# pyg-team/pytorch_geometric

Measured on AMD Instinct MI355X. Metric: edges/sec (fwd+bwd) 3-layer SAGE, ogbn-products shape, higher is better.
Workload: dtype f32

## Files before the change

pytorch_geometric_amd/_native.py:

```python
import collections
import ctypes
import os
import threading
from typing import Optional, Tuple

import torch
from torch import Tensor

from . import _compiled, _lib
from ._lib import REDUCE_IDS, PygAmdError, SpmmArgs, check

HUB_THRESHOLD = 1024
HUB_CHUNK = int(os.environ.get('PYGAMD_HUB_CHUNK', '256'))


def _require_device(*tensors):
    for t in tensors:
        if t is not None and not t.is_cuda:
            raise PygAmdError(
                'pytorch_geometric_amd kernels need HIP device tensors (got a '
                f'{t.device} tensor); there is no CPU fallback on this path')


def _idx_dtype(t: Tensor) -> int:
# ... 1375 lines not shown


SAGE_FUSED_VARIANT = int(os.environ.get('PYGAMD_FUSED_VARIANT', '0'))
SAGE_FUSED_PROBE = 0
AGG_GIVEN = _lib.AGG_GIVEN


def sage_layer_forward(rowptr: Tensor, col: Tensor, x_gather: Tensor, x_root: Tensor, w: Tensor,
                       bias: Optional[Tensor], reduce: str, relu: bool, agg: Tensor, out: Tensor,
                       hub=None, save_agg=True, hub_threshold: int = None,
                       hub_chunk: int = None, relu_bits: Optional[Tensor] = None,
                       mask_bits: Optional[Tensor] = None, row_scale: Optional[Tensor] = None,
                       out_scaled: Optional[Tensor] = None, variant: Optional[int] = None,
                       gather_width: Optional[int] = None,
                       compressed_out: Optional[Tensor] = None,
                       rowend: Optional[Tensor] = None) -> Tensor:
    _require_device(rowptr, col, x_gather, x_root, w, bias, agg, out, relu_bits, mask_bits,
                    row_scale, out_scaled, compressed_out)
    variant = SAGE_FUSED_VARIANT if variant is None else variant
    given = not isinstance(save_agg, bool) and int(save_agg) == AGG_GIVEN
    save_agg = AGG_GIVEN if given else int(bool(save_agg))
    if given:
        if gather_width is not None:
            raise ValueError("'save_agg=AGG_GIVEN' reads dense aggregated rows: not with a "
                             "compressed 'x_gather'")
        hub = None
    lab = bool(variant or SAGE_FUSED_PROBE)
    C = None if lab else _compiled.ops()
    if (C is not None and gather_width is None and compressed_out is None and rowend is None
            and _plain(x_gather, x_root, w, agg, out, out_scaled)):
        n_rows, F, Fo = rowptr.numel() - 1, x_gather.size(1), w.size(0)
        ok = (x_root.shape == (n_rows, F) and w.size(1) == 2 * F and agg.shape == (n_rows, F)
              and out.shape == (n_rows, Fo)
              and (out_scaled is None or (row_scale is not None and row_scale.numel() == n_rows
                                          and row_scale.dtype == torch.float32
                                          and out_scaled.shape == (n_rows, Fo)
                                          and (Fo <= 1 or out_scaled.stride(1) == 1))))
        if ok:
            _check_bits(relu_bits, n_rows, Fo)
            _check_bits(mask_bits, n_rows, Fo)
            h_rows, h_cptr, n_hub, n_chunks = _hub4(hub)
            with _timed({'n_rows': n_rows, 'n_src': x_gather.size(0),
                         'nnz': 0 if given else col.numel(), 'F': F,
                         'reduce': reduce, 'idx_bytes': rowptr.element_size(), 'weighted': False,
                         'src_scale': False, 'accumulate': False, 'n_hub': n_hub,
                         'fused_gemm': {'Fo': Fo, 'K': 2 * F, 'save_agg': bool(save_agg),
                                        'backward': mask_bits is not None,
                                        'scaled_copy': out_scaled is not None}}, x_gather):
                if given:
                    C.sage_layer_given(rowptr, x_root, w, bias, REDUCE_IDS[reduce], relu, agg,
                                       out, relu_bits, mask_bits, row_scale, out_scaled)
                else:
                    C.sage_layer_fused(
                        rowptr, col, x_gather, x_root, w, bias, REDUCE_IDS[reduce], relu, agg,
                        out, h_rows, h_cptr, n_hub, n_chunks,
                        HUB_THRESHOLD if hub_threshold is None else hub_threshold,
                        HUB_CHUNK if hub_chunk is None else hub_chunk, save_agg, relu_bits,
                        mask_bits, row_scale, out_scaled)
            return out
    lib = _lib.load_lab() if lab else _lib.load()
    xr, w2 = _f32_rows(x_root, 'x_root'), _f32_rows(w, 'weight')
    if gather_width is None:
        xg = _f32_rows(x_gather, 'x')
        F = xg.size(1)
    else:
        _check_compressed(x_gather, gather_width, 'x_gather')
        xg, F = x_gather, gather_width
    n_rows, Fo = rowptr.numel() - 1, w2.size(0)
    if rowend is not None:
        _require_device(rowend)
        n_rows = xr.size(0)
        if rowend.dtype != rowptr.dtype or not rowend.is_contiguous() \
                or rowend.numel() < n_rows or rowptr.numel() < n_rows:
            raise ValueError("'rowend' needs the dtype of 'rowptr' and one entry per row")
    if xr.shape != (n_rows, F) or w2.size(1) != 2 * F or agg.shape != (n_rows, F) \
            or out.shape != (n_rows, Fo):
        raise ValueError('shape mismatch in sage_layer_forward')
    a = SpmmArgs()
    a.rowptr, a.col = rowptr.data_ptr(), col.data_ptr()
    if rowend is not None:
        a.rowend = rowend.data_ptr()
    a.x, a.out = xg.data_ptr(), agg.data_ptr()
    a.n_rows, a.n_src, a.F = n_rows, xg.size(0), F
    a.ldx, a.ldo = _ld(xg), _ld(agg)
    a.idx_dtype, a.reduce = _idx_dtype(rowptr), REDUCE_IDS[reduce]
    a.w_heads, a.head_dim = 1, F
    if gather_width is not None:
        a.x_format = _lib.X_COMPRESSED
    if hub is not None and hub[2] > 0:
        hub_rows, hub_cptr, n_hub, n_chunks = hub
        a.hub_rows, a.hub_chunk_ptr = hub_rows.data_ptr(), hub_cptr.data_ptr()
        a.n_hub, a.n_chunks = n_hub, n_chunks
        a.hub_threshold = HUB_THRESHOLD if hub_threshold is None else hub_threshold
        a.hub_chunk = HUB_CHUNK if hub_chunk is None else hub_chunk
    if bias is not None:
        bias = bias.contiguous()
    _check_bits(relu_bits, n_rows, Fo)
    _check_bits(mask_bits, n_rows, Fo)
    f = _lib.SageFusedArgs()
    f.x_root, f.ld_root = xr.data_ptr(), _ld(xr)
    f.w, f.ldw = w2.data_ptr(), _ld(w2)
# ... 27 lines not shown
    check(lib.pygamd_sage_layer_fused_workspace_bytes(ctypes.byref(a), ctypes.byref(f),
                                                      ctypes.byref(nbytes)))
    ws_bytes = nbytes.value
    ws = torch.empty(ws_bytes, dtype=torch.uint8, device=xg.device) if ws_bytes else None
    if lab:
        check(lib.pygamd_lab_sage_layer_fused(ctypes.byref(a), ctypes.byref(f), variant or 1,
                                              SAGE_FUSED_PROBE, _p(ws), ws_bytes, _stream(xg)),
              'sage_layer_forward (lab schedule)')
    else:
        check(lib.pygamd_sage_layer_fused(ctypes.byref(a), ctypes.byref(f), _p(ws), ws_bytes,
                                          _stream(xg)), 'sage_layer_forward')
    if sink is not None:
        ev1.record(torch.cuda.current_stream(xg.device))
        sink.append(({'n_rows': n_rows, 'n_src': xg.size(0),
                      'nnz': 0 if given else col.numel(), 'F': F,
                      'reduce': reduce, 'idx_bytes': rowptr.element_size(), 'weighted': False,
                      'src_scale': False, 'accumulate': False, 'n_hub': a.n_hub,
                      'compressed_src': gather_width is not None,
                      'fused_gemm': {'Fo': Fo, 'K': 2 * F, 'save_agg': bool(save_agg),
                                     'backward': mask_bits is not None,
                                     'scaled_copy': out_scaled is not None,
                                     'compressed_out': compressed_out is not None}}, ev0, ev1))
    return out


def cross_entropy_rows(logits: Tensor, target: Tensor, index: Optional[Tensor] = None):
    _require_device(logits, target, index)
    x = _f32_rows(logits, 'logits')
    N, C = x.shape
    if target.dtype != torch.int64 or target.dim() != 1 or target.numel() != N \
            or not target.is_contiguous():
# ... 891 lines not shown
```

pytorch_geometric_amd/csrc/sage_fused.hip:

```cpp
#include "sage_fused_device.h"

namespace pygamd {

template <typename IdxT, int LPR, bool ZSRC = false, bool GIVEN = false>
__global__ void __launch_bounds__(kFBlock, 4)
    sage_fused_fwd_kernel(SageFusedArgs<IdxT> a) {
  extern __shared__ __align__(16) float smem[];
  __shared__ int next_row;
  __shared__ uint32_t zw[kFWaves * 32];
  const int agg_ld = a.f_pad + 4;
  float* agg = smem;
  float* xr = smem + kFTile * agg_ld;
  const int lane = lane_id();
  const int wave = __builtin_amdgcn_readfirstlane(static_cast<int>(threadIdx.x >> 6));
  const int64_t tile = xcd_logical_block();
  const int64_t row0 = tile * kFTile;
  if (row0 >= a.g.n_rows) return;

  if (!GIVEN && threadIdx.x == 0) next_row = 0;
  fused_stage_root<IdxT>(a, smem, xr, agg_ld, row0);
  if constexpr (GIVEN) {
    fused_stage_given<IdxT>(a, agg, agg_ld, row0);
  } else {
    __syncthreads();
    for (;;) {
      int r = 0;
      if (lane == 0) r = atomicAdd(&next_row, 1);
      r = __builtin_amdgcn_readfirstlane(r);
      if (r >= kFTile) break;
      fused_gather_row<IdxT, 4, LPR, ZSRC>(a, row0 + r, agg + r * agg_ld, lane);
    }
  }
  __syncthreads();
  fused_transform<IdxT, 1>(a, agg, xr, agg_ld, row0, wave, lane, a.zout ? zw : nullptr);
}

constexpr int kPK = 16;

inline int split_f_half(int64_t F) {
  return static_cast<int>(F <= 128 ? round_up(F, kPK) : round_up(F, 4 * kPK));
}
inline size_t split_planes_bytes(int64_t F, int64_t Fo) {
  const size_t steps = static_cast<size_t>(2 * split_f_half(F) / kPK);
  return static_cast<size_t>(ceil_div(Fo, 32)) * steps * 3 * kWave * sizeof(u32x4);
}
// ... 32 lines not shown
  for (int t = 0; t < 3; ++t) dst[t * kWave] = t3[t];
}

__device__ __forceinline__ void split_store4(uint32_t* __restrict__ p, int pstride, float x0,
                                             float x1, float x2, float x3) {
  uint32_t ta[3], tb[3];
  split_pair(x0, x1, ta);
  split_pair(x2, x3, tb);
#pragma unroll
  for (int t = 0; t < 3; ++t) {
    const u32x2 v = {ta[t], tb[t]};
    *reinterpret_cast<u32x2*>(p + t * pstride) = v;
  }
}

template <typename IdxT, int LPR>
__device__ __forceinline__ void split_gather_row(const SageFusedArgs<IdxT>& a, int64_t row,
                                                 uint32_t* __restrict__ prow, int pstride,
                                                 int lane) {
  constexpr int VW = 4, CH = 1;
  int fo[CH], head[CH];
  bool fv[CH];
  const int lir = lane % LPR;
  fo[0] = lir * VW;
  fv[0] = fo[0] < a.g.F;
  head[0] = 0;
  float acc[CH][VW];
#pragma unroll
  for (int i = 0; i < VW; ++i) acc[0][i] = 0.f;
  IdxT start = 0, end = 0;
  if (row < a.g.n_rows) {
    start = a.g.rowptr[row];
    end = spmm_row_end(a.g, row);
  }
  const IdxT deg = end - start;
  const bool hub = a.g.hub_threshold > 0 && deg > a.g.hub_threshold;
  if (hub) {
    if (lane < LPR && fv[0]) {
      const Vec<VW> v = load_vec<VW>(a.g.out + row * a.g.ldo + fo[0]);
      split_store4(prow + (fo[0] >> 1), pstride, v.v[0], v.v[1], v.v[2], v.v[3]);
    }
    return;
  }
  spmm_accumulate<IdxT, VW, LPR, CH, 0, false>(a.g, start, end, lane, fo, fv, head, acc);
  combine_subgroups<VW, LPR, CH>(acc);
  if (lane < LPR && fv[0]) {
    const float cntf = static_cast<float>(deg > 0 ? deg : 1);
    float o[VW];
#pragma unroll
    for (int i = 0; i < VW; ++i) o[i] = a.g.mean ? acc[0][i] / cntf : acc[0][i];
    split_store4(prow + (fo[0] >> 1), pstride, o[0], o[1], o[2], o[3]);
    if (a.save_agg && row < a.g.n_rows) {
#pragma unroll
      for (int i = 0; i < VW; ++i)
        __builtin_nontemporal_store(o[i], a.g.out + row * a.g.ldo + fo[0] + i);
    }
  }
}

// ... 35 lines not shown
        }
      }
      __builtin_amdgcn_sched_barrier(0);
      int sn = s + q + D;
      sn = sn < last ? sn : last;
#pragma unroll
      for (int t = 0; t < 3; ++t) rb[q][t] = wq[(sn * 3 + t) * kWave];
#pragma unroll
      for (int t = 0; t < 3; ++t) fa[t] = fan[t];
      __builtin_amdgcn_sched_barrier(0);
    }
  }
}

template <typename IdxT, int LPR, int NPASS, bool PROBE, bool OCC3 = (NPASS == 1),
          bool GIVEN = false>
__global__ void __launch_bounds__(kFBlock, OCC3 ? 6 : 4)
    sage_fused_split_kernel(SageFusedArgs<IdxT> a) {
  constexpr int D = OCC3 ? 2 : 4;
  constexpr int NU = 4;
  extern __shared__ __align__(16) uint32_t pl[];
  __shared__ int next_row;
  const int F = static_cast<int>(a.g.F);
  const int fh = a.f_half;
  const int KT = NPASS == 1 ? 2 * fh : fh;
  const int row_dw = KT / 2 + 4;
  const int pstride = kFTile * row_dw;
  const int lane = lane_id();
  const int wave = __builtin_amdgcn_readfirstlane(static_cast<int>(threadIdx.x >> 6));
  const int64_t tile = xcd_logical_block();
  const int64_t row0 = tile * kFTile;
// ... 56 lines not shown
    for (int i = 0; i < NU; ++i) {
      const int t = threadIdx.x + i * kFBlock;
      const int r = t / units;
      const int u = t - r * units;
      if (t < kFTile * units)
        split_store4(pl + r * row_dw + 2 * u, pstride, ga[i][0], ga[i][1], ga[i][2], ga[i][3]);
    }
  } else {
    __syncthreads();

    for (; !(PROBE && (a.probe & 1));) {
      int r = 0;
      if (lane == 0) r = atomicAdd(&next_row, 1);
      r = __builtin_amdgcn_readfirstlane(r);
      if (r >= kFTile) break;
      split_gather_row<IdxT, LPR>(a, row0 + r, pl + r * row_dw, pstride, lane);
    }
  }
  __syncthreads();

  const int wave_col0 = wave * 32;
  const bool active = wave_col0 < a.Fo && !(PROBE && (a.probe & 2));
  const int li = lane & 31, lh = lane >> 5;
  const int steps = 2 * fh / kPK;
  const u32x4* __restrict__ wq = a.wp + static_cast<int64_t>(wave) * steps * 3 * kWave + lane;
  const uint32_t* aq = pl + li * row_dw + 4 * lh;
  f32x16 acc0, acc1;
#pragma unroll
  for (int e = 0; e < 16; ++e) acc0[e] = acc1[e] = 0.f;
  if constexpr (NPASS == 1) {
    if (active) split_pass<D>(wq, aq, pstride, steps, acc0, acc1);
// ... 8 lines not shown
  if (wave_col0 >= a.Fo) return;
#pragma unroll
  for (int e = 0; e < 16; ++e) acc0[e] += acc1[e];
  f32x16 vout;
  fused_epilogue<IdxT>(a, acc0, row0, wave_col0, lane, vout);
}

template <typename IdxT, int LPR>
static int launch_fused(const SageFusedArgs<IdxT>& a, hipStream_t st, bool zsrc) {
  const size_t lds = sizeof(float) * 2 * kFTile * (a.f_pad + 4);
  void (*k)(SageFusedArgs<IdxT>) = sage_fused_fwd_kernel<IdxT, LPR, false>;
  if constexpr (LPR == kWave) {
    if (zsrc) k = sage_fused_fwd_kernel<IdxT, LPR, true>;
  }
  if (a.save_agg == PYGAMD_AGG_GIVEN) k = sage_fused_fwd_kernel<IdxT, LPR, false, true>;
  PYGAMD_HIP_CHECK(hipFuncSetAttribute(reinterpret_cast<const void*>(k),
                                       hipFuncAttributeMaxDynamicSharedMemorySize,
                                       static_cast<int>(lds)));
  const int64_t tiles = ceil_div(a.g.n_rows, kFTile);
  const unsigned grid = static_cast<unsigned>(round_up(tiles, 8));
  hipLaunchKernelGGL(k, dim3(grid), dim3(kFBlock), lds, st, a);
  PYGAMD_LAUNCH_CHECK();
  return PYGAMD_OK;
}

template <typename IdxT, int LPR, int NPASS>
static int launch_split(const SageFusedArgs<IdxT>& a, hipStream_t st) {
  const int KT = NPASS == 1 ? 2 * a.f_half : a.f_half;
  const size_t lds = sizeof(uint32_t) * 3 * kFTile * (KT / 2 + 4);
  void (*k)(SageFusedArgs<IdxT>) = a.probe ? sage_fused_split_kernel<IdxT, LPR, NPASS, true>
                                           : sage_fused_split_kernel<IdxT, LPR, NPASS, false>;
  if constexpr (NPASS == 2) {
    if (a.probe & 16) k = sage_fused_split_kernel<IdxT, LPR, NPASS, true, true>;
  }
  if (a.save_agg == PYGAMD_AGG_GIVEN)
    k = sage_fused_split_kernel<IdxT, LPR, NPASS, false, NPASS == 1, true>;
  PYGAMD_HIP_CHECK(hipFuncSetAttribute(reinterpret_cast<const void*>(k),
                                       hipFuncAttributeMaxDynamicSharedMemorySize,
                                       static_cast<int>(lds)));
  const int64_t tiles = ceil_div(a.g.n_rows, kFTile);
  const unsigned grid = static_cast<unsigned>(round_up(tiles, 8));
  hipLaunchKernelGGL(k, dim3(grid), dim3(kFBlock), lds, st, a);
  PYGAMD_LAUNCH_CHECK();
  return PYGAMD_OK;
}

static bool split_eligible(const pygamd_spmm_args* graph, const pygamd_sage_fused_args* f) {
  return pygamd_get_gemm_mode() == PYGAMD_GEMM_SPLIT_BF16 && graph->x_format == PYGAMD_X_DENSE &&
         !f->compressed_out;
}

// ... 114 lines not shown
```

pytorch_geometric_amd/csrc/sage_fused_device.h:

```cpp
#pragma once
#include "spmm_device.h"
#include "split_bf16.h"

namespace pygamd {

typedef float f32x16 __attribute__((ext_vector_type(16)));
typedef float f32x4 __attribute__((ext_vector_type(4)));

constexpr int kFTile = 32;
constexpr int kFBlock = 512;
constexpr int kFWaves = kFBlock / kWave;
constexpr int kFK = 32;
constexpr int kFLD = kFK + 4;
constexpr int kFMaxFo = 256;

template <typename IdxT>
struct SageFusedArgs {
  SpmmDev<IdxT> g;
  const float* __restrict__ x_root;
  int64_t ld_root;
  const float* __restrict__ w;
  int64_t ldw;
  const float* __restrict__ bias;
  float* __restrict__ y;
// ... 181 lines not shown
        if (c + PF < n_chunks && !(a.probe & 16)) load_b(c + PF, ring[q]);
        chunk(c);
      }
    }
  }

  if (dual) {
#pragma unroll
    for (int e = 0; e < 16; ++e) acc[e] += acc2[e];
  }
  f32x16 vout;
  fused_epilogue<IdxT>(a, acc, row0, wave_col0, lane, vout);
  if (zw) fused_compress_tile<IdxT>(a, vout, zw, row0, wave, lane, true);
}

template <typename IdxT, int VW, int LPR, bool ZSRC = false>
__device__ __forceinline__ void fused_gather_row(const SageFusedArgs<IdxT>& a, int64_t row,
                                                 float* __restrict__ agg_row, int lane) {
  constexpr int CH = 1;
  int fo[CH], head[CH];
  bool fv[CH];
  const int lir = lane % LPR;
  fo[0] = lir * VW;
  fv[0] = fo[0] < a.g.F;
  head[0] = 0;
  float acc[CH][VW];
#pragma unroll
  for (int i = 0; i < VW; ++i) acc[0][i] = 0.f;
  IdxT start = 0, end = 0;
  if (row < a.g.n_rows) {
    start = a.g.rowptr[row];
    end = spmm_row_end(a.g, row);
  }
  const IdxT deg = end - start;
  const bool hub = a.g.hub_threshold > 0 && deg > a.g.hub_threshold;
  if (hub) {
    if (lane < LPR && fv[0]) {
      const Vec<VW> v = load_vec<VW>(a.g.out + row * a.g.ldo + fo[0]);
      store_vec<VW>(agg_row + fo[0], v);
    }
    return;
  }
  spmm_accumulate<IdxT, VW, LPR, CH, ZSRC ? 4 : 0, false>(a.g, start, end, lane, fo, fv, head,
                                                          acc);
  combine_subgroups<VW, LPR, CH>(acc);
  if (lane < LPR && fv[0]) {
    const float cntf = static_cast<float>(deg > 0 ? deg : 1);
    Vec<VW> o;
#pragma unroll
    for (int i = 0; i < VW; ++i) o.v[i] = a.g.mean ? acc[0][i] / cntf : acc[0][i];
    store_vec<VW>(agg_row + fo[0], o);
    if (a.save_agg && row < a.g.n_rows) {
#pragma unroll
      for (int i = 0; i < VW; ++i)
        __builtin_nontemporal_store(o.v[i], a.g.out + row * a.g.ldo + fo[0] + i);
    }
  }
}
template <typename IdxT>
// ... 39 lines not shown
inline int sage_fused_lpr(int64_t F) {
  int lpr = 4;
  while (lpr < 64 && lpr * 4 < F) lpr <<= 1;
  return lpr;
}

inline int sage_fused_validate(const pygamd_spmm_args* graph, const pygamd_sage_fused_args* f,
                               bool* run) {
  *run = false;
  if (!graph || !f) return PYGAMD_ERR_INVALID_ARG;
  const int64_t F = graph->F, Fo = f->Fo;
  const bool given = f->save_agg == PYGAMD_AGG_GIVEN;
  if (graph->n_rows < 0 || F < 0 || Fo < 0 || (!given && graph->ldx < F) || graph->ldo < F ||
      f->ld_root < F || f->ldw < 2 * F || f->ldy < Fo)
    return PYGAMD_ERR_INVALID_ARG;
  if (!pygamd_sage_layer_forward_supported(F, Fo, graph->reduce) || graph->w ||
      graph->src_scale || graph->eid || graph->accumulate || graph->relu_mask ||
      graph->relu_bits)
    return PYGAMD_ERR_UNSUPPORTED;
  const int64_t words = (Fo + 31) / 32;
  if (f->relu_bits_out && (!f->relu || f->ld_bits_out < words)) return PYGAMD_ERR_INVALID_ARG;
  if (f->mask_bits && f->ld_mask_bits < words) return PYGAMD_ERR_INVALID_ARG;
  if (f->y_scaled && (!f->row_scale || f->ldy_scaled < Fo)) return PYGAMD_ERR_INVALID_ARG;
  const bool zsrc = graph->x_format == PYGAMD_X_COMPRESSED;
  if (graph->x_format != PYGAMD_X_DENSE && !zsrc) return PYGAMD_ERR_INVALID_ARG;
  if (given && zsrc) return PYGAMD_ERR_UNSUPPORTED;
  if (graph->rowend && (graph->n_hub > 0 || zsrc)) return PYGAMD_ERR_UNSUPPORTED;
  if (graph->accumulate_rows != 0) return PYGAMD_ERR_INVALID_ARG;
  if (zsrc && (graph->ldx < F + 12 || graph->src_bits)) return PYGAMD_ERR_INVALID_ARG;
  if (f->compressed_out && (Fo % 32 != 0 || f->ld_compressed < Fo + 12))
    return PYGAMD_ERR_INVALID_ARG;
  if (graph->n_rows == 0) return PYGAMD_OK;
  if ((!given && (!graph->rowptr || !graph->x)) || !graph->out || !f->x_root || !f->w || !f->y)
// ... 12 lines not shown
                               size_t workspace_bytes, void* stream) {
  if (graph->n_hub <= 0) return PYGAMD_OK;
  pygamd_spmm_args hubs = *graph;
  hubs.hub_phase = 2;
  return pygamd_spmm_csr(&hubs, workspace, workspace_bytes, stream);
}

template <typename IdxT>
inline SageFusedArgs<IdxT> sage_fused_fill(const pygamd_spmm_args* graph,
                                           const pygamd_sage_fused_args* f) {
  SageFusedArgs<IdxT> a;
  const int64_t F = graph->F;
  a.g.rowptr = static_cast<const IdxT*>(graph->rowptr);
  a.g.col = static_cast<const IdxT*>(graph->col);
  a.g.eid = nullptr;
  a.g.w = nullptr;
  a.g.src_scale = nullptr;
  a.g.x = graph->x;
  a.g.out = graph->out;
  a.g.arg_out = nullptr;
  a.g.arg32_out = nullptr;
  a.g.relu_mask = nullptr;
  a.g.ldm = 0;
  a.g.relu_bits = nullptr;
  a.g.ldb = 0;
  a.g.src_bits = nullptr;
  a.g.src_bits_set = nullptr;
  a.g.n_src = graph->n_src;
  a.g.n_rows = graph->n_rows;
  a.g.F = F;
  a.g.ldx = graph->ldx;
// ... 41 lines not shown
```

pytorch_geometric_amd/csrc/sage_fused_lab.hip:

```cpp
#include "sage_fused_device.h"
#include "../../include/pyg_amd_lab.h"

namespace pygamd {

template <typename IdxT, int LPR>
__global__ void __launch_bounds__(kFBlock, 4) sage_fused_probe_kernel(SageFusedArgs<IdxT> a) {
  extern __shared__ __align__(16) float smem[];
  __shared__ int next_row;
  const int agg_ld = a.f_pad + 4;
  float* agg = smem;
  float* xr = smem + kFTile * agg_ld;
  const int lane = lane_id();
  const int wave = __builtin_amdgcn_readfirstlane(static_cast<int>(threadIdx.x >> 6));
  const int64_t tile = xcd_logical_block();
  const int64_t row0 = tile * kFTile;
  if (row0 >= a.g.n_rows) return;
  fused_stage_root<IdxT>(a, smem, xr, agg_ld, row0);
  if (threadIdx.x == 0) next_row = 0;
  __syncthreads();
  if (a.probe & 2048) __builtin_amdgcn_s_setprio(2);
  for (; !(a.probe & 1);) {
    int r = 0;
    if (lane == 0) r = atomicAdd(&next_row, 1);
    r = __builtin_amdgcn_readfirstlane(r);
// ... 547 lines not shown
#undef PYGAMD_LAB_COPY
  PYGAMD_LAUNCH_CHECK();
  return PYGAMD_OK;
}

extern "C" int pygamd_lab_sage_layer_fused(const pygamd_spmm_args* graph,
                                           const pygamd_sage_fused_args* f, int variant,
                                           int probe, void* workspace, size_t workspace_bytes,
                                           void* stream) {
  bool run = false;
  int rc = sage_fused_validate(graph, f, &run);
  if (rc != PYGAMD_OK || !run) return rc;
  if (variant < 1 || variant > 6) return PYGAMD_ERR_INVALID_ARG;
  if (variant == 5) return sage_layer_fused_run(graph, f, true, probe, workspace, workspace_bytes, stream);
  if (variant == 6) return sage_layer_fused_run(graph, f, false, 0, workspace, workspace_bytes, stream);
  if (graph->x_format != PYGAMD_X_DENSE || f->compressed_out || f->save_agg == PYGAMD_AGG_GIVEN)
    return PYGAMD_ERR_UNSUPPORTED;
  if (graph->rowend && variant != 5 && variant != 6 && variant != 1) return PYGAMD_ERR_UNSUPPORTED;
  hipStream_t st = as_stream(stream);
  rc = sage_fused_hub_pass(graph, workspace, workspace_bytes, stream);
  if (rc != PYGAMD_OK) return rc;
  const bool streamed = variant == 2 && graph->n_src < (static_cast<int64_t>(1) << 31);
  const int spec_nm = variant == 3 ? 4 : variant == 4 ? 8 : 0;
  const int lpr = sage_fused_lpr(graph->F);
  return PYGAMD_DISPATCH_IDX(graph->idx_dtype, [&]() -> int {
    SageFusedArgs<IdxT> a = sage_fused_fill<IdxT>(graph, f);
    a.probe = probe;
    if (spec_nm) {
      switch (lpr) {
        case 4: return launch_spec<IdxT, 4>(a, spec_nm, st);
        case 8: return launch_spec<IdxT, 8>(a, spec_nm, st);
// ... 15 lines not shown
```

pytorch_geometric_amd/csrc/torch_binding.cpp:

```cpp
#include <ATen/ATen.h>
#include <ATen/hip/impl/HIPGuardImplMasqueradingAsCUDA.h>
#include <c10/hip/HIPStream.h>
#include <torch/csrc/autograd/custom_function.h>
#include <torch/library.h>

#include "../../include/pyg_amd.h"

namespace {

using at::Tensor;
using OptTensor = c10::optional<Tensor>;

inline void* ptr(const Tensor& t) { return t.defined() ? t.data_ptr() : nullptr; }
inline void* ptr(const OptTensor& t) {
  return (t.has_value() && t->defined()) ? t->data_ptr() : nullptr;
}
inline const float* fptr(const Tensor& t) { return static_cast<const float*>(ptr(t)); }
inline bool has(const OptTensor& t) { return t.has_value() && t->defined(); }

inline void* cur_stream(const Tensor& ref) {
  return c10::hip::getCurrentHIPStream(ref.get_device()).stream();
}

inline int idx_dtype(const Tensor& t) {
// ... 194 lines not shown
                        g2.options().dtype(at::kByte));
  check(pygamd_linear_wgrad2(fptr(g2), ld(g2), fptr(first), ld(first), K1, fptr(second),
                             second.defined() ? ld(second) : 0, K2, M, N, accumulate ? 1 : 0,
                             static_cast<int>(wgs_per_cu), static_cast<float*>(ptr(out)), ld(out),
                             static_cast<float*>(ptr(grad_b)), ptr(ws), nbytes, cur_stream(g2)),
        "linear_wgrad");
}

void sage_layer_fused(const Tensor& rowptr, const OptTensor& col, const Tensor& x_gather,
                        const Tensor& x_root, const Tensor& w, const OptTensor& bias,
                        int64_t reduce, bool relu, Tensor agg, Tensor out,
                        const OptTensor& hub_rows, const OptTensor& hub_cptr, int64_t n_hub,
                        int64_t n_chunks, int64_t hub_threshold, int64_t hub_chunk,
                        int64_t save_agg ,
                        const OptTensor& relu_bits, const OptTensor& mask_bits,
                        const OptTensor& row_scale, const OptTensor& out_scaled) {
  const c10::hip::HIPGuardMasqueradingAsCUDA device_guard(rowptr.device());
  check_index(rowptr, rowptr, "rowptr");
  check_index(col, rowptr, "col");
  check_index(hub_rows, rowptr, "hub_rows");
  check_index(hub_cptr, rowptr, "hub_chunk_ptr");
  const Tensor xg = rows_f32(x_gather, "x"), xr = rows_f32(x_root, "x_root");
  const Tensor w2 = rows_f32(w, "weight");
  const int64_t n_rows = rowptr.numel() - 1, F = xg.size(1), Fo = w2.size(0);
  TORCH_CHECK(xr.size(0) == n_rows && xr.size(1) == F && w2.size(1) == 2 * F &&
                  agg.size(0) == n_rows && agg.size(1) == F && out.size(0) == n_rows &&
                  out.size(1) == Fo,
              "shape mismatch in sage_layer_forward");
  pygamd_spmm_args a = {};
  a.rowptr = ptr(rowptr);
  a.col = ptr(col);
  a.x = fptr(xg);
  a.out = static_cast<float*>(ptr(agg));
  a.n_rows = n_rows;
  a.n_src = xg.size(0);
  a.F = F;
  a.ldx = ld(xg);
  a.ldo = ld(agg);
  a.idx_dtype = idx_dtype(rowptr);
  a.reduce = static_cast<int32_t>(reduce);
  a.w_heads = 1;
  a.head_dim = static_cast<int32_t>(F);
  if (n_hub > 0 && has(hub_rows) && has(hub_cptr)) {
    a.hub_rows = ptr(hub_rows);
    a.hub_chunk_ptr = ptr(hub_cptr);
    a.n_hub = n_hub;
    a.n_chunks = n_chunks;
    a.hub_threshold = hub_threshold;
    a.hub_chunk = hub_chunk;
  }
  const Tensor b = contig(bias), rs = contig(row_scale);
  pygamd_sage_fused_args f = {};
  f.x_root = fptr(xr);
  f.ld_root = ld(xr);
  f.w = fptr(w2);
  f.ldw = ld(w2);
  f.bias = fptr(b);
// ... 23 lines not shown
  }
  size_t ws_bytes = 0;
  check(pygamd_sage_layer_fused_workspace_bytes(&a, &f, &ws_bytes), "sage_layer_forward");
  Tensor ws;
  if (ws_bytes > 0)
    ws = at::empty({static_cast<int64_t>(ws_bytes)}, xg.options().dtype(at::kByte));
  check(pygamd_sage_layer_fused(&a, &f, ptr(ws), ws_bytes, cur_stream(xg)), "sage_layer_forward");
}

void sage_layer_given(const Tensor& rowptr, const Tensor& x_root, const Tensor& w,
                      const OptTensor& bias, int64_t reduce, bool relu, const Tensor& agg,
                      Tensor out, const OptTensor& relu_bits, const OptTensor& mask_bits,
                      const OptTensor& row_scale, const OptTensor& out_scaled) {
  sage_layer_fused(rowptr, OptTensor(), x_root, x_root, w, bias, reduce, relu, agg, out,
                   OptTensor(), OptTensor(), 0, 0, 0, 0, PYGAMD_AGG_GIVEN, relu_bits, mask_bits,
                   row_scale, out_scaled);
}

Tensor index2ptr(const Tensor& index, int64_t size) {
  const c10::hip::HIPGuardMasqueradingAsCUDA device_guard(index.device());
  const Tensor idx = index.contiguous();
  Tensor out = at::empty({size + 1}, idx.options());
  check(pygamd_index2ptr(ptr(idx), idx_dtype(idx), idx.numel(), size, ptr(out), cur_stream(idx)),
        "index2ptr");
  return out;
}

Tensor ptr2index(const Tensor& p, int64_t n) {
  const c10::hip::HIPGuardMasqueradingAsCUDA device_guard(p.device());
  const Tensor pc = p.contiguous();
  Tensor out = at::empty({n}, pc.options());
// ... 242 lines not shown
      "int hub_phase, Tensor(b!)? arg32, Tensor? relu_mask, Tensor? relu_bits) -> ()");
  m.def(
      "linear_forward(Tensor x, Tensor w, Tensor? bias, bool relu, Tensor(a!) out, "
      "bool accumulate) -> ()");
  m.def(
      "linear_dgrad(Tensor g, Tensor w_t, Tensor? row_scale, int n_scaled, Tensor(a!) out, "
      "bool accumulate, Tensor? relu_mask, Tensor? relu_bits, Tensor(b!)? out_scaled) -> ()");
  m.def(
      "linear_wgrad(Tensor g, Tensor x, Tensor(a!) out, bool accumulate, int wgs_per_cu, "
      "Tensor(b!)? grad_b, Tensor? x2) -> ()");
  m.def(
      "sage_layer_fused(Tensor rowptr, Tensor? col, Tensor x_gather, Tensor x_root, Tensor w, "
      "Tensor? bias, int reduce, bool relu, Tensor(a!) agg, Tensor(b!) out, Tensor? hub_rows, "
      "Tensor? hub_cptr, int n_hub, int n_chunks, int hub_threshold, int hub_chunk, "
      "int save_agg, Tensor(c!)? relu_bits, Tensor? mask_bits, Tensor? row_scale, "
      "Tensor(d!)? out_scaled) -> ()");
  m.def(
      "sage_layer_given(Tensor rowptr, Tensor x_root, Tensor w, Tensor? bias, int reduce, "
      "bool relu, Tensor agg, Tensor(a!) out, Tensor(b!)? relu_bits, Tensor? mask_bits, "
      "Tensor? row_scale, Tensor(c!)? out_scaled) -> ()");
  m.def("index2ptr(Tensor index, int size) -> Tensor");
  m.def("ptr2index(Tensor ptr, int n) -> Tensor");
  m.def("gather_rows(Tensor x, Tensor index) -> Tensor");
  m.def(
      "gather_scatter_add(Tensor x, Tensor gather_idx, Tensor scatter_idx, Tensor? scale, "
      "Tensor? w, Tensor(a!) out, Tensor? n_valid) -> ()");
  m.def(
      "sddmm_csr(Tensor rowptr, Tensor? col, Tensor? eid, Tensor grad_out, Tensor x, "
      "int n_edges, int w_heads) -> Tensor");
  m.def("segment_softmax_forward(Tensor src, Tensor ptr) -> Tensor");
  m.def("segment_softmax_backward(Tensor out, Tensor grad_out, Tensor ptr) -> Tensor");
// ... 75 lines not shown
```

pytorch_geometric_amd/edge_index.py:

```python
import weakref
from typing import Optional, Tuple

import torch
from torch import Tensor

from . import _native


class CSR:

    def __init__(self, ptr: Tensor, idx: Tensor, perm: Tensor, n_rows: int, n_cols: int):
        self.ptr, self.idx, self.perm = ptr, idx, perm
        self.n_rows, self.n_cols = n_rows, n_cols
        self._hub = None
        self._inv_deg = None
        self._agg0 = None

    @property
    def hub(self):
        if self._hub is None:
            self._hub = _native.hub_plan(self.ptr)
        return self._hub

    @property
    def nnz(self) -> int:
        return self.idx.numel()

    def degree(self) -> Tensor:
        return self.ptr[1:] - self.ptr[:-1]

    def inv_degree(self) -> Tensor:
        if self._inv_deg is None:
            self._inv_deg = 1.0 / self.degree().clamp(min=1).to(torch.float32)
        return self._inv_deg


def build_csr(key: Tensor, other: Tensor, n_rows: int, n_cols: int,
              is_sorted: bool = False) -> CSR:
    if is_sorted:
        perm = torch.arange(key.numel(), dtype=key.dtype, device=key.device)
        ptr = _native.index2ptr(key, n_rows)
        return CSR(ptr, other.contiguous(), perm, n_rows, n_cols)
    sorted_key, perm64 = _native.index_sort(key, max_value=max(n_rows - 1, 0))
    idx = _native.permute_index(other, perm64)
    ptr = _native.index2ptr(sorted_key, n_rows)
    perm = _native.cast_index(perm64, key.dtype)
    return CSR(ptr, idx, perm, n_rows, n_cols)


# ... 72 lines not shown
    @classmethod
    def from_sorted_batch(cls, edge_index: Tensor, num_nodes: int,
                          max_in_degree: Optional[int] = None) -> 'EdgeIndex':
        self = cls(edge_index, (num_nodes, num_nodes), sort_order='col', validate=False)
        self.atomic_backward = True
        csr = self.by_dst()
        if max_in_degree is not None and max_in_degree <= _native.HUB_THRESHOLD:
            csr._hub = (None, None, 0, 0)
        return self

    def record_stream(self, stream) -> None:
        tensors = [self.edge_index]
        for csr in (self._csr, self._csc):
            if csr is not None:
                tensors += [csr.ptr, csr.idx, csr.perm, csr._inv_deg]
                if csr._hub is not None:
                    tensors += [csr._hub[0], csr._hub[1]]
        for t in tensors:
            if isinstance(t, Tensor) and t.is_cuda:
                t.record_stream(stream)

    def trim(self, num_nodes: int, num_edges: int) -> 'EdgeIndex':
        ei = self.edge_index.narrow(1, 0, num_edges)
        if self.sort_order != 'col' or self._csr is None:
            out = EdgeIndex(ei, (num_nodes, num_nodes), sort_order=self.sort_order,
                            validate=False)
            out.atomic_backward = self.atomic_backward
            return out
        out = EdgeIndex(ei, (num_nodes, num_nodes), sort_order='col', validate=False)
        out.atomic_backward = self.atomic_backward
# ... 187 lines not shown
```

pytorch_geometric_amd/nn/models/_fused_sage.py:

```python
import os
import threading
import weakref
from typing import List, Optional

import torch
from torch import Tensor
from torch.autograd import Function

from ... import _native
from ...edge_index import EdgeIndex

RELU_EPILOGUE = os.environ.get('PYGAMD_RELU_EPILOGUE', '1') != '0'
GEMM_BACKEND = os.environ.get('PYGAMD_GEMM', 'own')
FUSE_LAYER = os.environ.get('PYGAMD_FUSE_LAYER', '1') != '0'
FUSE_BWD = os.environ.get('PYGAMD_FUSE_BWD', '1') != '0'
OVERLAP_WGRAD = os.environ.get('PYGAMD_OVERLAP_WGRAD', '0') != '0'
OVERLAP_WGS = int(os.environ.get('PYGAMD_OVERLAP_WGS', '1'))
COMPRESS_ROWS = os.environ.get('PYGAMD_COMPRESS_ROWS', '0') != '0'
SPARSE_GRAD = os.environ.get('PYGAMD_SPARSE_GRAD', '1') != '0'
_agg0_handles = weakref.WeakSet()
_call = threading.local()


def cache_agg0_enabled() -> bool:
    return os.environ.get('PYGAMD_CACHE_AGG0', '1') != '0'


def clear_aggregation_cache() -> None:
    for handle in list(_agg0_handles):
        handle._agg0 = None
    _agg0_handles.clear()


def _agg0_key(x: Tensor, aggr: str):
    return (x._version, x.data_ptr(), tuple(x.shape), tuple(x.stride()), aggr,
            _native.HUB_THRESHOLD, _native.HUB_CHUNK)
# ... 203 lines not shown
        g = grad_out
        if g.dim() != 2 or g.stride(1) != 1 or (g.size(0) > 1 and g.stride(0) < g.size(1)):
            g = g.contiguous()
        grad_x = None
        pending = []
        own = GEMM_BACKEND == 'own'
        masked = True
        needs_in = [layer > 0 or ctx.needs_input_grad[0] for layer in range(L)]

        def fused_bwd(layer: int) -> bool:
            Fi, Fo = ctx.dims[layer]
            return (own and FUSE_BWD and FUSE_LAYER and ctx.modes[layer] == 'post'
                    and needs_in[layer] and (layer == 0 or bits[layer] is not None)
                    and _native.sage_layer_forward_supported(Fo, Fi, 'sum'))

        g_scaled = None
        for layer in reversed(range(L)):
            buf, wmat = bufs[layer], wmats[layer]
            Fi, Fo = ctx.dims[layer]
            want_b = ctx.has_bias[layer]
            if not masked:
                h_next = FusedSageStack._input_view(ctx, bufs, layer + 1)
                g, grads[3 * layer + 1] = _native.relu_backward_colsum(g, h_next, want_b)
                g_scaled = None
            elif want_b and not own:
                grads[3 * layer + 1] = _native.colsum(g)
            need_input_grad = needs_in[layer]
            mask_in = FusedSageStack._input_view(ctx, bufs, layer) if (own and layer > 0) else None
            bits_in = bits[layer] if mask_in is not None else None
            mask_f = mask_in if bits_in is None else None
            scaled_for_next = layer > 0 and scale is not None and fused_bwd(layer - 1)
            if ctx.modes[layer] == 'post':
                one_launch = fused_bwd(layer) and g.stride(0) % 4 == 0 and g.data_ptr() % 16 == 0
                overlap = (own and OVERLAP_WGRAD and need_input_grad and not one_launch
                           and not torch.cuda.is_current_stream_capturing())
                lone_x = x0 if layer == 0 else None
                overlap_one = (own and OVERLAP_WGRAD and one_launch
                               and not torch.cuda.is_current_stream_capturing())
                if overlap_one:
                    cur = torch.cuda.current_stream(g.device)
                    side = _side_stream(g.device)
                    side.wait_stream(cur)
                    with torch.cuda.stream(side):
                        gw = _native.linear_wgrad(g, buf, wgs_per_cu=OVERLAP_WGS, bias_grad=want_b,
                                                  x2=lone_x)
                        if want_b:
                            gw, grads[3 * layer + 1] = gw
                    for t in (g, buf) + ((lone_x, ) if lone_x is not None else ()):
                        t.record_stream(side)
                    pending.append(side)
                elif not overlap:
                    if own:
                        gw = _native.linear_wgrad(g, buf, bias_grad=want_b, x2=lone_x)
                        if want_b:
                            gw, grads[3 * layer + 1] = gw
                    else:
                        gw = torch.mm(g.t(), buf)
                if one_launch:
                    if scale is None:
                        gsrc = g
                    elif g_scaled is not None:
                        gsrc = g_scaled
                    else:
                        gsrc = g * scale.view(-1, 1)
                    wc = torch.cat([wmat[:, :Fi].t(), wmat[:, Fi:].t()], dim=1)
                    gin = torch.empty(N, Fi, dtype=torch.float32, device=g.device)
                    gin_s = torch.empty_like(gin) if scaled_for_next else None
                    scratch = gin if Fi == Fo else torch.empty(N, Fo, dtype=torch.float32,
                                                               device=g.device)
                    _native.sage_layer_forward(bwd.ptr, bwd.idx, gsrc, g, wc, None, 'sum', False,
                                               scratch, gin, hub=bwd.hub, save_agg=False,
                                               mask_bits=bits_in,
                                               row_scale=scale if gin_s is not None else None,
                                               out_scaled=gin_s)
                    grads[3 * layer] = gw[:, :Fi]
                    grads[3 * layer + 2] = gw[:, Fi:]
                    g, g_scaled = gin, gin_s
                    masked = mask_in is not None
                    if layer == 0:
                        grad_x = g
                    continue
                if need_input_grad:
                    if own:
                        gcat = _native.linear_dgrad(g, wmat.t().contiguous(), scale,
                                                    Fi if scale is not None else 0)
                        pre_scaled = True
                    else:
                        gcat = torch.mm(g, wmat)
                        pre_scaled = False
# ... 196 lines not shown
```

Measured before the change: 4.586 billion.

## Use per-slot inverse-degree edge weights in fused SAGE backward gather

The fused backward gather now multiplies each neighbour by a per-edge inverse-degree weight (cached per CSR, gathered from the inverse-degree vector). This replaces the pre-scaled gradient copy (out_scaled / g*scale) that the next layer previously consumed. The aim is to drop the extra scaled-output write and the separate scaling pass. In exchange the gather reads one extra float per edge, and the weighted accumulate path may unroll differently.

```diff
diff --git a/pytorch_geometric_amd/_native.py b/pytorch_geometric_amd/_native.py
--- a/pytorch_geometric_amd/_native.py
+++ b/pytorch_geometric_amd/_native.py
@@ -1413,9 +1413,17 @@
                        out_scaled: Optional[Tensor] = None, variant: Optional[int] = None,
                        gather_width: Optional[int] = None,
                        compressed_out: Optional[Tensor] = None,
-                       rowend: Optional[Tensor] = None) -> Tensor:
+                       rowend: Optional[Tensor] = None,
+                       slot_weights: Optional[Tensor] = None) -> Tensor:
     _require_device(rowptr, col, x_gather, x_root, w, bias, agg, out, relu_bits, mask_bits,
-                    row_scale, out_scaled, compressed_out)
+                    row_scale, out_scaled, compressed_out, slot_weights)
+    if slot_weights is not None:
+        if slot_weights.dtype != torch.float32 or slot_weights.dim() != 1 \
+                or slot_weights.numel() != col.numel():
+            raise ValueError(f"'slot_weights' must hold one float32 per slot of 'col' "
+                             f"({col.numel()}), got {slot_weights.dtype} "
+                             f"{tuple(slot_weights.shape)}")
+        slot_weights = slot_weights.contiguous()
     variant = SAGE_FUSED_VARIANT if variant is None else variant
     given = not isinstance(save_agg, bool) and int(save_agg) == AGG_GIVEN
     save_agg = AGG_GIVEN if given else int(bool(save_agg))
@@ -1423,6 +1431,8 @@
         if gather_width is not None:
             raise ValueError("'save_agg=AGG_GIVEN' reads dense aggregated rows: not with a "
                              "compressed 'x_gather'")
+        if slot_weights is not None:
+            raise ValueError("'slot_weights' weigh a gather: not with 'save_agg=AGG_GIVEN'")
         hub = None
     lab = bool(variant or SAGE_FUSED_PROBE)
     C = None if lab else _compiled.ops()
@@ -1441,7 +1451,8 @@
             h_rows, h_cptr, n_hub, n_chunks = _hub4(hub)
             with _timed({'n_rows': n_rows, 'n_src': x_gather.size(0),
                          'nnz': 0 if given else col.numel(), 'F': F,
-                         'reduce': reduce, 'idx_bytes': rowptr.element_size(), 'weighted': False,
+                         'reduce': reduce, 'idx_bytes': rowptr.element_size(),
+                         'weighted': slot_weights is not None,
                          'src_scale': False, 'accumulate': False, 'n_hub': n_hub,
                          'fused_gemm': {'Fo': Fo, 'K': 2 * F, 'save_agg': bool(save_agg),
                                         'backward': mask_bits is not None,
@@ -1455,7 +1466,7 @@
                         out, h_rows, h_cptr, n_hub, n_chunks,
                         HUB_THRESHOLD if hub_threshold is None else hub_threshold,
                         HUB_CHUNK if hub_chunk is None else hub_chunk, save_agg, relu_bits,
-                        mask_bits, row_scale, out_scaled)
+                        mask_bits, row_scale, out_scaled, slot_weights)
             return out
     lib = _lib.load_lab() if lab else _lib.load()
     xr, w2 = _f32_rows(x_root, 'x_root'), _f32_rows(w, 'weight')
@@ -1484,6 +1495,8 @@
     a.ldx, a.ldo = _ld(xg), _ld(agg)
     a.idx_dtype, a.reduce = _idx_dtype(rowptr), REDUCE_IDS[reduce]
     a.w_heads, a.head_dim = 1, F
+    if slot_weights is not None:
+        a.w = slot_weights.data_ptr()
     if gather_width is not None:
         a.x_format = _lib.X_COMPRESSED
     if hub is not None and hub[2] > 0:
@@ -1541,7 +1554,8 @@
         ev1.record(torch.cuda.current_stream(xg.device))
         sink.append(({'n_rows': n_rows, 'n_src': xg.size(0),
                       'nnz': 0 if given else col.numel(), 'F': F,
-                      'reduce': reduce, 'idx_bytes': rowptr.element_size(), 'weighted': False,
+                      'reduce': reduce, 'idx_bytes': rowptr.element_size(),
+                      'weighted': slot_weights is not None,
                       'src_scale': False, 'accumulate': False, 'n_hub': a.n_hub,
                       'compressed_src': gather_width is not None,
                       'fused_gemm': {'Fo': Fo, 'K': 2 * F, 'save_agg': bool(save_agg),
diff --git a/pytorch_geometric_amd/csrc/sage_fused.hip b/pytorch_geometric_amd/csrc/sage_fused.hip
--- a/pytorch_geometric_amd/csrc/sage_fused.hip
+++ b/pytorch_geometric_amd/csrc/sage_fused.hip
@@ -2,7 +2,7 @@
 
 namespace pygamd {
 
-template <typename IdxT, int LPR, bool ZSRC = false, bool GIVEN = false>
+template <typename IdxT, int LPR, bool ZSRC = false, bool GIVEN = false, bool WSLOT = false>
 __global__ void __launch_bounds__(kFBlock, 4)
     sage_fused_fwd_kernel(SageFusedArgs<IdxT> a) {
   extern __shared__ __align__(16) float smem[];
@@ -28,7 +28,7 @@
       if (lane == 0) r = atomicAdd(&next_row, 1);
       r = __builtin_amdgcn_readfirstlane(r);
       if (r >= kFTile) break;
-      fused_gather_row<IdxT, 4, LPR, ZSRC>(a, row0 + r, agg + r * agg_ld, lane);
+      fused_gather_row<IdxT, 4, LPR, ZSRC, WSLOT>(a, row0 + r, agg + r * agg_ld, lane);
     }
   }
   __syncthreads();
@@ -91,7 +91,7 @@
   }
 }
 
-template <typename IdxT, int LPR>
+template <typename IdxT, int LPR, bool WSLOT = false>
 __device__ __forceinline__ void split_gather_row(const SageFusedArgs<IdxT>& a, int64_t row,
                                                  uint32_t* __restrict__ prow, int pstride,
                                                  int lane) {
@@ -119,7 +119,10 @@
     }
     return;
   }
-  spmm_accumulate<IdxT, VW, LPR, CH, 0, false>(a.g, start, end, lane, fo, fv, head, acc);
+  constexpr int UF =
+      (WSLOT && LPR < kWave && LPR >= 8) ? ((LPR == 8 && sizeof(IdxT) == 8) ? 2 : 4) : 0;
+  spmm_accumulate<IdxT, VW, LPR, CH, WSLOT ? 1 : 0, false, UF>(a.g, start, end, lane, fo, fv, head,
+                                                               acc);
   combine_subgroups<VW, LPR, CH>(acc);
   if (lane < LPR && fv[0]) {
     const float cntf = static_cast<float>(deg > 0 ? deg : 1);
@@ -185,7 +188,7 @@
 }
 
 template <typename IdxT, int LPR, int NPASS, bool PROBE, bool OCC3 = (NPASS == 1),
-          bool GIVEN = false>
+          bool GIVEN = false, bool WSLOT = false>
 __global__ void __launch_bounds__(kFBlock, OCC3 ? 6 : 4)
     sage_fused_split_kernel(SageFusedArgs<IdxT> a) {
   constexpr int D = OCC3 ? 2 : 4;
@@ -272,7 +275,7 @@
       if (lane == 0) r = atomicAdd(&next_row, 1);
       r = __builtin_amdgcn_readfirstlane(r);
       if (r >= kFTile) break;
-      split_gather_row<IdxT, LPR>(a, row0 + r, pl + r * row_dw, pstride, lane);
+      split_gather_row<IdxT, LPR, WSLOT>(a, row0 + r, pl + r * row_dw, pstride, lane);
     }
   }
   __syncthreads();
@@ -311,6 +314,7 @@
     if (zsrc) k = sage_fused_fwd_kernel<IdxT, LPR, true>;
   }
   if (a.save_agg == PYGAMD_AGG_GIVEN) k = sage_fused_fwd_kernel<IdxT, LPR, false, true>;
+  if (a.g.w) k = sage_fused_fwd_kernel<IdxT, LPR, false, false, true>;
   PYGAMD_HIP_CHECK(hipFuncSetAttribute(reinterpret_cast<const void*>(k),
                                        hipFuncAttributeMaxDynamicSharedMemorySize,
                                        static_cast<int>(lds)));
@@ -332,6 +336,8 @@
   }
   if (a.save_agg == PYGAMD_AGG_GIVEN)
     k = sage_fused_split_kernel<IdxT, LPR, NPASS, false, NPASS == 1, true>;
+  if (a.g.w)
+    k = sage_fused_split_kernel<IdxT, LPR, NPASS, false, NPASS == 1, false, true>;
   PYGAMD_HIP_CHECK(hipFuncSetAttribute(reinterpret_cast<const void*>(k),
                                        hipFuncAttributeMaxDynamicSharedMemorySize,
                                        static_cast<int>(lds)));
diff --git a/pytorch_geometric_amd/csrc/sage_fused_device.h b/pytorch_geometric_amd/csrc/sage_fused_device.h
--- a/pytorch_geometric_amd/csrc/sage_fused_device.h
+++ b/pytorch_geometric_amd/csrc/sage_fused_device.h
@@ -219,7 +219,7 @@
   if (zw) fused_compress_tile<IdxT>(a, vout, zw, row0, wave, lane, true);
 }
 
-template <typename IdxT, int VW, int LPR, bool ZSRC = false>
+template <typename IdxT, int VW, int LPR, bool ZSRC = false, bool WSLOT = false>
 __device__ __forceinline__ void fused_gather_row(const SageFusedArgs<IdxT>& a, int64_t row,
                                                  float* __restrict__ agg_row, int lane) {
   constexpr int CH = 1;
@@ -246,8 +246,9 @@
     }
     return;
   }
-  spmm_accumulate<IdxT, VW, LPR, CH, ZSRC ? 4 : 0, false>(a.g, start, end, lane, fo, fv, head,
-                                                          acc);
+  static_assert(!(ZSRC && WSLOT), "slot weights: dense source rows only");
+  spmm_accumulate<IdxT, VW, LPR, CH, WSLOT ? 1 : (ZSRC ? 4 : 0), false>(a.g, start, end, lane, fo,
+                                                                        fv, head, acc);
   combine_subgroups<VW, LPR, CH>(acc);
   if (lane < LPR && fv[0]) {
     const float cntf = static_cast<float>(deg > 0 ? deg : 1);
@@ -317,9 +318,10 @@
   if (graph->n_rows < 0 || F < 0 || Fo < 0 || (!given && graph->ldx < F) || graph->ldo < F ||
       f->ld_root < F || f->ldw < 2 * F || f->ldy < Fo)
     return PYGAMD_ERR_INVALID_ARG;
-  if (!pygamd_sage_layer_forward_supported(F, Fo, graph->reduce) || graph->w ||
-      graph->src_scale || graph->eid || graph->accumulate || graph->relu_mask ||
-      graph->relu_bits)
+  if (!pygamd_sage_layer_forward_supported(F, Fo, graph->reduce) || graph->src_scale ||
+      graph->eid || graph->accumulate || graph->relu_mask || graph->relu_bits)
+    return PYGAMD_ERR_UNSUPPORTED;
+  if (graph->w && (graph->w_heads != 1 || given || graph->x_format != PYGAMD_X_DENSE))
     return PYGAMD_ERR_UNSUPPORTED;
   const int64_t words = (Fo + 31) / 32;
   if (f->relu_bits_out && (!f->relu || f->ld_bits_out < words)) return PYGAMD_ERR_INVALID_ARG;
@@ -362,7 +364,7 @@
   a.g.rowptr = static_cast<const IdxT*>(graph->rowptr);
   a.g.col = static_cast<const IdxT*>(graph->col);
   a.g.eid = nullptr;
-  a.g.w = nullptr;
+  a.g.w = graph->w;
   a.g.src_scale = nullptr;
   a.g.x = graph->x;
   a.g.out = graph->out;
diff --git a/pytorch_geometric_amd/csrc/sage_fused_lab.hip b/pytorch_geometric_amd/csrc/sage_fused_lab.hip
--- a/pytorch_geometric_amd/csrc/sage_fused_lab.hip
+++ b/pytorch_geometric_amd/csrc/sage_fused_lab.hip
@@ -585,7 +585,8 @@
   if (variant < 1 || variant > 6) return PYGAMD_ERR_INVALID_ARG;
   if (variant == 5) return sage_layer_fused_run(graph, f, true, probe, workspace, workspace_bytes, stream);
   if (variant == 6) return sage_layer_fused_run(graph, f, false, 0, workspace, workspace_bytes, stream);
-  if (graph->x_format != PYGAMD_X_DENSE || f->compressed_out || f->save_agg == PYGAMD_AGG_GIVEN)
+  if (graph->x_format != PYGAMD_X_DENSE || f->compressed_out ||
+      f->save_agg == PYGAMD_AGG_GIVEN || graph->w)
     return PYGAMD_ERR_UNSUPPORTED;
   if (graph->rowend && variant != 5 && variant != 6 && variant != 1) return PYGAMD_ERR_UNSUPPORTED;
   hipStream_t st = as_stream(stream);
diff --git a/pytorch_geometric_amd/csrc/torch_binding.cpp b/pytorch_geometric_amd/csrc/torch_binding.cpp
--- a/pytorch_geometric_amd/csrc/torch_binding.cpp
+++ b/pytorch_geometric_amd/csrc/torch_binding.cpp
@@ -232,7 +232,8 @@
                         int64_t n_chunks, int64_t hub_threshold, int64_t hub_chunk,
                         int64_t save_agg ,
                         const OptTensor& relu_bits, const OptTensor& mask_bits,
-                        const OptTensor& row_scale, const OptTensor& out_scaled) {
+                        const OptTensor& row_scale, const OptTensor& out_scaled,
+                        const OptTensor& slot_weights) {
   const c10::hip::HIPGuardMasqueradingAsCUDA device_guard(rowptr.device());
   check_index(rowptr, rowptr, "rowptr");
   check_index(col, rowptr, "col");
@@ -259,6 +260,13 @@
   a.reduce = static_cast<int32_t>(reduce);
   a.w_heads = 1;
   a.head_dim = static_cast<int32_t>(F);
+  const Tensor sw = contig(slot_weights);
+  if (sw.defined()) {
+    TORCH_CHECK(has(col) && sw.scalar_type() == at::kFloat && sw.numel() == col->numel() &&
+                    sw.device() == xg.device(),
+                "'slot_weights' must hold one float32 per slot of 'col'");
+    a.w = fptr(sw);
+  }
   if (n_hub > 0 && has(hub_rows) && has(hub_cptr)) {
     a.hub_rows = ptr(hub_rows);
     a.hub_chunk_ptr = ptr(hub_cptr);
@@ -312,7 +320,7 @@
                       const OptTensor& row_scale, const OptTensor& out_scaled) {
   sage_layer_fused(rowptr, OptTensor(), x_root, x_root, w, bias, reduce, relu, agg, out,
                    OptTensor(), OptTensor(), 0, 0, 0, 0, PYGAMD_AGG_GIVEN, relu_bits, mask_bits,
-                   row_scale, out_scaled);
+                   row_scale, out_scaled, OptTensor());
 }
 
 Tensor index2ptr(const Tensor& index, int64_t size) {
@@ -585,7 +593,7 @@
       "Tensor? bias, int reduce, bool relu, Tensor(a!) agg, Tensor(b!) out, Tensor? hub_rows, "
       "Tensor? hub_cptr, int n_hub, int n_chunks, int hub_threshold, int hub_chunk, "
       "int save_agg, Tensor(c!)? relu_bits, Tensor? mask_bits, Tensor? row_scale, "
-      "Tensor(d!)? out_scaled) -> ()");
+      "Tensor(d!)? out_scaled, Tensor? slot_weights) -> ()");
   m.def(
       "sage_layer_given(Tensor rowptr, Tensor x_root, Tensor w, Tensor? bias, int reduce, "
       "bool relu, Tensor agg, Tensor(a!) out, Tensor(b!)? relu_bits, Tensor? mask_bits, "
diff --git a/pytorch_geometric_amd/edge_index.py b/pytorch_geometric_amd/edge_index.py
--- a/pytorch_geometric_amd/edge_index.py
+++ b/pytorch_geometric_amd/edge_index.py
@@ -15,6 +15,7 @@
         self._hub = None
         self._inv_deg = None
         self._agg0 = None
+        self._slot_inv_deg = None
 
     @property
     def hub(self):
@@ -33,6 +34,14 @@
         if self._inv_deg is None:
             self._inv_deg = 1.0 / self.degree().clamp(min=1).to(torch.float32)
         return self._inv_deg
+
+    def slot_inv_degree(self, inv_deg: Tensor) -> Tensor:
+        hit = self._slot_inv_deg
+        if hit is not None and hit[0] is inv_deg and hit[1] == inv_deg._version:
+            return hit[2]
+        w = inv_deg.to(torch.float32)[self.idx]
+        self._slot_inv_deg = (inv_deg, inv_deg._version, w)
+        return w
 
 
 def build_csr(key: Tensor, other: Tensor, n_rows: int, n_cols: int,
@@ -135,6 +144,8 @@
         for csr in (self._csr, self._csc):
             if csr is not None:
                 tensors += [csr.ptr, csr.idx, csr.perm, csr._inv_deg]
+                if csr._slot_inv_deg is not None:
+                    tensors.append(csr._slot_inv_deg[2])
                 if csr._hub is not None:
                     tensors += [csr._hub[0], csr._hub[1]]
         for t in tensors:
diff --git a/pytorch_geometric_amd/nn/models/_fused_sage.py b/pytorch_geometric_amd/nn/models/_fused_sage.py
--- a/pytorch_geometric_amd/nn/models/_fused_sage.py
+++ b/pytorch_geometric_amd/nn/models/_fused_sage.py
@@ -20,6 +20,10 @@
 SPARSE_GRAD = os.environ.get('PYGAMD_SPARSE_GRAD', '1') != '0'
 _agg0_handles = weakref.WeakSet()
 _call = threading.local()
+
+
+def slot_weights_enabled() -> bool:
+    return os.environ.get('PYGAMD_SLOT_WEIGHTS', '1') != '0'
 
 
 def cache_agg0_enabled() -> bool:
@@ -253,6 +257,8 @@
                     and needs_in[layer] and (layer == 0 or bits[layer] is not None)
                     and _native.sage_layer_forward_supported(Fo, Fi, 'sum'))
 
+        slot_w = (slot_weights_enabled() and scale is not None
+                  and hasattr(bwd, 'slot_inv_degree'))
         g_scaled = None
         for layer in reversed(range(L)):
             buf, wmat = bufs[layer], wmats[layer]
@@ -268,7 +274,8 @@
             mask_in = FusedSageStack._input_view(ctx, bufs, layer) if (own and layer > 0) else None
             bits_in = bits[layer] if mask_in is not None else None
             mask_f = mask_in if bits_in is None else None
-            scaled_for_next = layer > 0 and scale is not None and fused_bwd(layer - 1)
+            scaled_for_next = (layer > 0 and scale is not None and not slot_w
+                               and fused_bwd(layer - 1))
             if ctx.modes[layer] == 'post':
                 one_launch = fused_bwd(layer) and g.stride(0) % 4 == 0 and g.data_ptr() % 16 == 0
                 overlap = (own and OVERLAP_WGRAD and need_input_grad and not one_launch
@@ -296,7 +303,7 @@
                     else:
                         gw = torch.mm(g.t(), buf)
                 if one_launch:
-                    if scale is None:
+                    if scale is None or slot_w:
                         gsrc = g
                     elif g_scaled is not None:
                         gsrc = g_scaled
@@ -307,11 +314,12 @@
                     gin_s = torch.empty_like(gin) if scaled_for_next else None
                     scratch = gin if Fi == Fo else torch.empty(N, Fo, dtype=torch.float32,
                                                                device=g.device)
+                    weights = {'slot_weights': bwd.slot_inv_degree(scale)} if slot_w else {}
                     _native.sage_layer_forward(bwd.ptr, bwd.idx, gsrc, g, wc, None, 'sum', False,
                                                scratch, gin, hub=bwd.hub, save_agg=False,
                                                mask_bits=bits_in,
                                                row_scale=scale if gin_s is not None else None,
-                                               out_scaled=gin_s)
+                                               out_scaled=gin_s, **weights)
                     grads[3 * layer] = gw[:, :Fi]
                     grads[3 * layer + 2] = gw[:, Fi:]
                     g, g_scaled = gin, gin_s
```

Result: no change. 4.560 billion (-0.6%).
